# DonsetPG/graph-physics

Hardware: AMD Instinct MI355X
Metric: training steps/sec, CylinderFlow 15-round MGN (batch 16 meshes per step) (higher is better)
Workload: dtype f32; 1 GPU; BASELINE.json configs[1], fp32: 16 x 1885-node CylinderFlow-like meshes per GPU (N=30160, E=180082), 15 rounds, latent 128, random init; global_batch_meshes=16, launch=eager, parallelism=single

## Files before the change

graph-physics_amd/_capi.py:

```python
from __future__ import annotations

import ctypes as C
import os
import subprocess
import threading

_HERE = os.path.dirname(os.path.abspath(__file__))
_CSRC = os.path.join(_HERE, "csrc")
_REPO = os.path.dirname(_HERE)
LIB_PATH = os.environ.get("MGN_LIB") or os.path.join(_CSRC, "libmgn_hip.so")
SOURCES = [os.path.join(_CSRC, "mgn_kernels.hip"), os.path.join(_CSRC, "mgn_prep.hip"), os.path.join(_CSRC, "mgn_attn.hip"),
           os.path.join(_CSRC, "mgn_dense.hip"), os.path.join(_CSRC, "mgn_loss.hip")]
DEPS = [os.path.join(_CSRC, "mgn_x6.inc"), os.path.join(_CSRC, "mgn_fused.inc"), os.path.join(_CSRC, "mgn_pp.inc"), os.path.join(_CSRC, "mgn_ppr.inc")]
HEADER = os.path.join(_REPO, "include", "mgn_hip.h")
DEVICE_FLAGS = ["-Xclang", "-target-feature", "-Xclang", "-packed-fp32-ops"]

MAX_LAYERS = 8
MAX_PHASES = 3
MAX_WGRAD_JOBS = 48

_f32p = C.c_void_p
_i32p = C.c_void_p


class MlpFwdArgs(C.Structure):
    _fields_ = [
        ("M", C.c_int64),
        ("H", C.c_int), ("NL", C.c_int), ("nphase", C.c_int),
        ("src", _f32p * MAX_PHASES),
        ("idx", _i32p * MAX_PHASES),
        ("kw", C.c_int * MAX_PHASES),
        ("W", _f32p * MAX_LAYERS),
        ("b", _f32p * MAX_LAYERS),
        ("scale", _f32p),
        ("eps", C.c_float),
# ... 210 lines not shown
    "mgn_sparse_attn_fwd_s": (C.c_int, [C.c_void_p, C.c_int64] * 3 + [C.c_int, C.c_void_p, C.c_void_p, C.c_int64, C.c_int, C.c_int] + [C.c_void_p] * 4),
    "mgn_sparse_attn_bwd_s": (C.c_int, [C.c_void_p, C.c_int64] * 3 + [C.c_int] + [C.c_void_p] * 8 + [C.c_int64, C.c_int64, C.c_int, C.c_int]
                              + [C.c_void_p, C.c_int64] * 3 + [C.c_void_p, C.c_size_t, C.c_void_p]),
    "mgn_sparse_attn_weights": (C.c_int, [C.c_void_p] * 6 + [C.c_int64, C.c_int, C.c_int, C.c_void_p, C.c_void_p]),
    "mgn_head_axis_attn_fwd": (C.c_int, [C.c_void_p] * 3 + [C.c_int64, C.c_int, C.c_int] + [C.c_void_p] * 3),
    "mgn_head_axis_attn_bwd": (C.c_int, [C.c_void_p] * 6 + [C.c_int64, C.c_int, C.c_int] + [C.c_void_p] * 4),
    "mgn_attn_last_error": (C.c_char_p, []),
    "mgn_linear_fwd": (C.c_int, [C.POINTER(LinearArgs), C.c_void_p]),
    "mgn_linear_accepts_transposed": (C.c_int, [C.c_int64, C.c_int, C.c_int, C.c_int, C.c_int]),
    "mgn_rownorm2_bwd": (C.c_int, [C.c_void_p, C.c_void_p, C.c_int, C.c_int, C.c_void_p, C.c_void_p, C.c_void_p, C.c_void_p, C.c_float, C.c_int64,
                                   C.c_void_p, C.c_void_p, C.c_void_p, C.c_void_p, C.c_size_t, C.c_void_p]),
    "mgn_act_gate_bwd": (C.c_int, [C.c_void_p, C.c_void_p, C.c_void_p, C.c_int64, C.c_int, C.c_int, C.c_int, C.c_void_p, C.c_void_p, C.c_void_p]),
    "mgn_rownorm_fwd": (C.c_int, [C.c_void_p, C.c_int, C.c_int, C.c_void_p, C.c_float, C.c_int64, C.c_void_p, C.c_void_p, C.c_void_p]),
    "mgn_rownorm_bwd_workspace_bytes": (C.c_size_t, [C.c_int]),
    "mgn_rownorm_bwd": (C.c_int, [C.c_void_p, C.POINTER(RownormPhase), C.c_int, C.c_void_p, C.c_void_p, C.c_float, C.c_int64, C.c_void_p,
                                  C.c_void_p, C.c_size_t, C.c_void_p]),
    "mgn_dense_last_error": (C.c_char_p, []),
    "mgn_loss_fd_geometry": (C.c_int, [C.c_void_p] * 4 + [C.c_int, C.c_int64, C.c_void_p, C.c_void_p, C.c_void_p]),
    "mgn_loss_ls_geometry": (C.c_int, [C.c_void_p, C.c_int64, C.c_int, C.c_void_p, C.c_int, C.c_int64] + [C.c_void_p] * 6),
    "mgn_loss_workspace_bytes": (C.c_size_t, []),
    "mgn_loss_fwd": (C.c_int, [C.POINTER(LossArgs), C.c_void_p]),
    "mgn_loss_bwd": (C.c_int, [C.POINTER(LossArgs)] + [C.c_void_p] * 5),
    "mgn_loss_last_error": (C.c_char_p, []),
}

_lib = None
_lock = threading.Lock()

EXPECTED_VERSION = 136
HASH_PATH = os.path.join(_CSRC, "libmgn_hip.srchash")
LOCK_PATH = os.path.join(_CSRC, ".build.lock")


def hipcc_path():
    for p in (os.environ.get("HIPCC"), "/opt/rocm/bin/hipcc"):
        if p and os.path.exists(p):
            return p
    from shutil import which

    return which("hipcc")


def source_hash() -> str:
    import hashlib

    h = hashlib.sha256()
# ... 57 lines not shown
            if needs_build():
                try:
                    build()
                except Exception as e:
                    raise RuntimeError(
                        f"MI355X engine library {LIB_PATH} is missing or older than its sources and could not be "
                        f"rebuilt ({e}); run `python -c 'import __graft_entry__ as g; g.build()'`") from e
            try:
                L = C.CDLL(LIB_PATH)
            except OSError as e:
                raise RuntimeError(f"cannot load {LIB_PATH}: {e}") from e
            for name, (res, args) in SYMBOLS.items():
                fn = getattr(L, name)
                fn.restype = res
                fn.argtypes = args
            v = L.mgn_version()
            if v != EXPECTED_VERSION:
                raise RuntimeError(f"{LIB_PATH} has ABI version {v}, this binding needs {EXPECTED_VERSION}: rebuild it "
                                   "(`python -c 'import __graft_entry__ as g; g.build()'`)")
            _lib = L
    return _lib


def check(rc: int, what: str, prep: bool = False, attn: bool = False, dense: bool = False, loss: bool = False):
    if rc != 0:
        fn = lib().mgn_loss_last_error if loss else lib().mgn_dense_last_error if dense else (lib().mgn_attn_last_error if attn else (lib().mgn_prep_last_error if prep else lib().mgn_last_error))
        msg = fn().decode("utf-8", "replace")
        raise RuntimeError(f"{what} failed (code {rc}): {msg}")
```

graph-physics_amd/csrc/mgn_prep.hip:

```cpp
#include <hip/hip_runtime.h>
#include <rocprim/device/device_radix_sort.hpp>
#include <rocprim/device/device_select.hpp>
#include <stdint.h>
#include <stdio.h>
#include "mgn_hip.h"

static thread_local char g_perr[256] = "";
extern "C" const char* mgn_prep_last_error(void) { return g_perr; }
static int pfail(int code, const char* msg) {
  snprintf(g_perr, sizeof(g_perr), "%s", msg);
  return code;
}
static int pcheck(const char* what) {
  hipError_t e = hipGetLastError();
  if (e != hipSuccess) {
    snprintf(g_perr, sizeof(g_perr), "%s: %s", what, hipGetErrorString(e));
    return 2;
  }
  return 0;
}

__global__ void k_face_keys(const int64_t* __restrict__ face, int K, long F, long N, uint64_t* __restrict__ keys, int* __restrict__ err) {
  const long f = (long)blockIdx.x * blockDim.x + threadIdx.x;
  if (f >= F) return;
// ... 351 lines not shown

__device__ __forceinline__ float sim_value(const mgn_sim_desc& d, int stream, long row, int col) {
  if (stream == 0) {
    const int nf = d.feat_end - d.feat_start;
    if (col < nf) return d.x[row * d.x_w + d.feat_start + col];
    const float t = d.x[row * d.x_w + d.type_idx];
    const int ti = (int)(long)t;
    if (col == nf && d.type_err != nullptr && (ti < 0 || ti >= MGN_NODE_TYPES)) *d.type_err = 1;
    return (ti == col - nf) ? 1.f : 0.f;
  }
  if (stream == 1) return d.y[row * d.y_w + col] - d.x[row * d.x_w + d.out_start + col];
  return d.edge_attr[row * d.edge_w + col];
}
__device__ __forceinline__ int sim_width(const mgn_sim_desc& d, int stream) {
  return stream == 0 ? (d.feat_end - d.feat_start) + MGN_NODE_TYPES : stream == 1 ? d.out_w : d.edge_w;
}
__device__ __forceinline__ long sim_rows(const mgn_sim_desc& d, int stream) { return stream == 2 ? d.E : d.N; }

__global__ void __launch_bounds__(256) k_stats_partial(const mgn_sim_desc d, float* __restrict__ part) {
  const int stream = blockIdx.y;
  if (!d.accumulate[stream] || !(*d.num_acc[stream] < d.max_accumulations)) return;
  const int W = sim_width(d, stream);
  const long M = sim_rows(d, stream);
  __shared__ float s1[256], s2[256];
  const int col = threadIdx.x % SIM_MAXW, rl = threadIdx.x / SIM_MAXW;
  float a = 0.f, b = 0.f;
  if (col < W)
    for (long r = (long)blockIdx.x * 8 + rl; r < M; r += (long)SIM_PART * 8) {
      const float v = sim_value(d, stream, r, col);
      a += v;
      b = fmaf(v, v, b);
    }
  s1[threadIdx.x] = a;
  s2[threadIdx.x] = b;
  __syncthreads();
  if (rl == 0) {
    for (int k = 1; k < 8; ++k) {
      a += s1[k * SIM_MAXW + col];
      b += s2[k * SIM_MAXW + col];
    }
    float* p = part + ((size_t)(stream * SIM_PART + blockIdx.x) * 2) * SIM_MAXW;
    p[col] = a;
    p[SIM_MAXW + col] = b;
  }
}

__global__ void __launch_bounds__(64) k_stats_final(const mgn_sim_desc d, const float* __restrict__ part) {
  const int stream = blockIdx.x;
  if (!d.accumulate[stream] || !(*d.num_acc[stream] < d.max_accumulations)) return;
  const int W = sim_width(d, stream);
  const int col = threadIdx.x % SIM_MAXW, which = threadIdx.x / SIM_MAXW;
  if (col < W) {
    float t = 0.f;
    for (int b = 0; b < SIM_PART; ++b) t += part[((size_t)(stream * SIM_PART + b) * 2 + which) * SIM_MAXW + col];
    float* dst = which == 0 ? d.acc_sum[stream] : d.acc_sumsq[stream];
    dst[col] += t;
  }
  if (threadIdx.x == 0) {
    *d.acc_count[stream] += (float)sim_rows(d, stream);
// ... 663 lines not shown
```

graph-physics_amd/ops.py:

```python
from __future__ import annotations

import ctypes as C
from typing import List, Optional, Sequence, Tuple

import torch

from . import _capi

EPS = 1e-8
import os as _os
X6_ENABLED = _os.environ.get("MGN_FP32_MFMA") is None

_matrix_precision = "fp32"


def set_matrix_precision(p: str) -> None:
    global _matrix_precision
    if p not in ("fp32", "bf16"):
        raise ValueError("matrix precision must be 'fp32' or 'bf16'")
    if p == "bf16" and not X6_ENABLED:
        raise RuntimeError("bf16 matrix mode runs on the split-bf16 kernels; unset MGN_FP32_MFMA")
    _matrix_precision = p


def get_matrix_precision() -> str:
    return _matrix_precision
SUPPORTED_H = (16, 32, 64, 128)


def _ptr(t: Optional[torch.Tensor]) -> Optional[int]:
    return None if t is None else t.data_ptr()


_raw_stream = getattr(torch._C, "_cuda_getCurrentRawStream", None)
# ... 452 lines not shown

def wpack(blocks: Sequence[Tuple[int, int, bool, int]], dev):
    if not blocks:
        return
    arr = (_capi.WpackBlock * len(blocks))()
    for i, (src, ld, tr, dst) in enumerate(blocks):
        arr[i].src, arr[i].ld_src, arr[i].transpose, arr[i].dst = src, ld, int(bool(tr)), dst
    with torch.cuda.device(dev):
        rc = _capi.lib().mgn_wpack(len(blocks), arr, _stream(dev))
    _capi.check(rc, "mgn_wpack")


def transpose_blocks(blocks: Sequence[Tuple[int, int, int, int]], H: int, dev):
    if not blocks:
        return
    arr = (_capi.TBlock * len(blocks))()
    for i, (src, lds, dst, ldd) in enumerate(blocks):
        arr[i].src, arr[i].ld_src, arr[i].dst, arr[i].ld_dst = src, lds, dst, ldd
    with torch.cuda.device(dev):
        rc = _capi.lib().mgn_transpose_blocks(len(blocks), arr, H, _stream(dev))
    _capi.check(rc, "mgn_transpose_blocks")


def gather_rows(src: torch.Tensor, idx: torch.Tensor, out: Optional[torch.Tensor] = None) -> torch.Tensor:
    n, H = int(idx.numel()), int(src.shape[1])
    if out is None:
        out = torch.empty(n, H, dtype=torch.float32, device=src.device)
    with torch.cuda.device(src.device):
        rc = _capi.lib().mgn_gather_rows(_ptr(src), _ptr(idx), n, H, _ptr(out), _stream(src.device))
    _capi.check(rc, "mgn_gather_rows", prep=True)
    return out


def halo_unpack_add(rows: torch.Tensor, nodes: torch.Tensor, rowptr: torch.Tensor, perm: torch.Tensor, dst: torch.Tensor):
    with torch.cuda.device(dst.device):
        rc = _capi.lib().mgn_halo_unpack_add(_ptr(rows), _ptr(nodes), _ptr(rowptr), _ptr(perm), int(nodes.numel()), int(dst.shape[1]),
                                             _ptr(dst), _stream(dst.device))
    _capi.check(rc, "mgn_halo_unpack_add", prep=True)


def gate_fwd(G, phi, gate_pos, agg, gate_out, agg_out):
    with torch.cuda.device(agg.device):
        rc = _capi.lib().mgn_gate_fwd(_ptr(G), _ptr(phi), _ptr(gate_pos), _ptr(agg), int(agg.shape[0]), int(agg.shape[1]),
                                      _ptr(gate_out), _ptr(agg_out), _stream(agg.device))
    _capi.check(rc, "mgn_gate_fwd", prep=True)

# ... 150 lines not shown
    fit = int(frac * free // max(per_round, 1))
    return max(0, L - fit)


class MlpFunction(torch.autograd.Function):

    @staticmethod
    def forward(ctx, x, has_norm, act, *params):
        _require_device(x, *params)
        x = _f32c(x)
        NL = (len(params) - (1 if has_norm else 0)) // 2
        Ws = [_f32c(params[2 * l]) for l in range(NL)]
        bs = [_f32c(params[2 * l + 1]) for l in range(NL)]
        scale = _f32c(params[2 * NL]) if has_norm else None
        if NL < 2:
            raise AssertionError("The MLP must have at least 2 layers (input and output).")
        M, kin = x.shape
        H = Ws[0].shape[0]
        out_w = Ws[-1].shape[0]
        if H not in SUPPORTED_H or kin > H or out_w > H:
            raise NotImplementedError(f"MLP widths (in={kin}, hidden={H}, out={out_w}) not supported by the MI355X engine")
        dev = x.device
        kp, op = pad16(kin), pad16(out_w)
        W0 = Ws[0]
        if kp != kin:
            W0 = torch.nn.functional.pad(W0, (0, kp - kin))
        Wl, bl = Ws[-1], bs[-1]
        if op != out_w:
            Wl = torch.nn.functional.pad(Wl, (0, 0, 0, op - out_w))
            bl = torch.nn.functional.pad(bl, (0, op - out_w))
        Wk = [W0] + Ws[1:-1] + [Wl]
        bk = bs[:-1] + [bl]
        prec = 1 if (_matrix_precision == "bf16" and not (H == 128 and out_w == H and X6_ENABLED and act != 2)) else 0
        if prec:
            Wk = [w.to(torch.bfloat16).to(torch.float32) for w in Wk]
            bk = [b.to(torch.bfloat16).to(torch.float32) for b in bk]
        need = any(ctx.needs_input_grad) and _saving()
        f = dict(dtype=torch.float32, device=dev)
        y = torch.empty(M, out_w, **f)
        x6 = H == 128 and out_w == H and X6_ENABLED and M > 0 and act != 2
        mode = "generic"
        if x6 and kin < H and 3 <= NL <= 4:
            mode = "enc"
        elif x6 and kin == H and NL <= 4:
            mode = "full"
        packed = mode != "generic"
        saveH = [torch.empty(M, H, **f) for _ in range(NL - 1)] if need else None
        U = torch.empty(M, H, **f) if (need and has_norm) else None
        R = torch.empty(M, **f) if (need and has_norm) else None
        Ms = [torch.empty(M, 4, dtype=torch.int32, device=dev) for _ in range(NL - 1)] if (need and packed and act == 0) else None
        Zs = [torch.empty(M, H, **f) for _ in range(NL - 1)] if (need and act != 0) else None
        if mode == "enc":
            h1 = saveH[0] if need else torch.empty(M, H, **f)
            mlp_fwd(M, H, [(x, None, kin)], [Wk[0]], [bk[0]], None, H, None, h1, Zs[0] if Zs else None, out_relu=True, act=act,
                    saveM=[Ms[0]] if Ms else None)
            pk = torch.empty((NL - 1) * _capi.WPACK_BYTES, dtype=torch.uint8, device=dev)
            units = [pk.data_ptr() + u * _capi.WPACK_BYTES for u in range(NL - 1)]
            wpack([(Wk[l + 1].data_ptr(), H, False, units[l]) for l in range(NL - 1)], dev)
            mlp_fwd(M, H, [(h1, None, H)], Wk[1:], bk[1:], scale, out_w, None, y, None,
                    saveH[1:] if need else None, U, R, wpk=units, saveM=Ms[1:] if Ms else None,
                    saveZ=Zs[1:] if Zs else None, act=act)
        elif mode == "full":
            pk = torch.empty(NL * _capi.WPACK_BYTES, dtype=torch.uint8, device=dev)
            units = [pk.data_ptr() + u * _capi.WPACK_BYTES for u in range(NL)]
            wpack([(Wk[l].data_ptr(), H, False, units[l]) for l in range(NL)], dev)
            mlp_fwd(M, H, [(x, None, H)], Wk, bk, scale, out_w, None, y, None, saveH, U, R, wpk=units, saveM=Ms, saveZ=Zs, act=act)
        else:
            mlp_fwd(M, H, [(x, None, kin)], Wk, bk, scale, out_w, None, y, None, saveH, U, R, act=act, saveZ=Zs, precision=prec)
        ctx.meta = (NL, H, kin, out_w, has_norm, kp != kin, op != out_w, act, mode)
        ctx.prec, ctx.Wk_rounded = prec, (Wk if prec else None)
        ctx.save_for_backward(x, *Ws, *([scale] if has_norm else []))
        ctx.pads = (W0 if kp != kin else None, Wl if op != out_w else None)
        ctx.saved_acts = (saveH, U, R, Ms, Zs)
        return y

    @staticmethod
    def backward(ctx, dy):
        NL, H, kin, out_w, has_norm, pad0, padl, act, mode = ctx.meta
        if ctx.saved_acts is None or ctx.saved_acts[0] is None:
            raise RuntimeError("MlpFunction: no saved activations -- backward ran a second time without retain_graph "
                               "support, or the forward ran under no_grad")
        t = ctx.saved_tensors
        x, Ws = t[0], list(t[1:1 + NL])
        scale = t[1 + NL] if has_norm else None
        Wk = [ctx.pads[0] if pad0 else Ws[0]] + Ws[1:-1] + [ctx.pads[1] if padl else Ws[-1]]
        prec = getattr(ctx, "prec", 0)
        if prec:
            Wk = ctx.Wk_rounded
        saveH, U, R, Ms, Zs = ctx.saved_acts
        dy = _f32c(dy)
        M, dev = x.shape[0], x.device
        kp, op = pad16(kin), pad16(out_w)
        f = dict(dtype=torch.float32, device=dev)
        widths = [H] * (NL - 1) + [op]
        zero = M == 0
        mk = torch.zeros if zero else torch.empty
        dZ = [mk(M, w, **f) for w in widths]
        db = [mk(w, **f) for w in widths]
        dscale = mk(H, **f) if has_norm else None
        dx = None
        want_dx = ctx.needs_input_grad[0]
        if want_dx and kin != H:
            raise NotImplementedError("input gradient of a ragged-width MLP input is not needed by the path")
        if want_dx:
            dx = mk(M, H, **f)
        if mode in ("enc", "full") and M > 0:
            tr = [Wk[l] for l in range(NL - 1, 0, -1)] + ([Wk[0]] if want_dx else [])
            pk = torch.empty(len(tr) * _capi.WPACK_BYTES, dtype=torch.uint8, device=dev)
            units = [pk.data_ptr() + u * _capi.WPACK_BYTES for u in range(len(tr))]
            wpack([(w.data_ptr(), H, True, units[u]) for u, w in enumerate(tr)], dev)
            din = [(None, None, dx)] if want_dx else []
            mlp_bwd(M, H, NL, dy, None, None, out_w, U, R, scale, saveH, [None] * NL, dZ, din, [None] * NL, dscale,
                    wpk=units, Ms=Ms, Zs=Zs, act=act)
        else:
            sq = [l for l in range(1, NL) if tuple(Wk[l].shape) == (H, H) and Wk[l].is_contiguous()]
            wt_buf = torch.empty(len(sq), H, H, **f) if sq else None
            if sq:
                transpose_blocks([(Wk[l].data_ptr(), H, wt_buf[k].data_ptr(), H) for k, l in enumerate(sq)], H, dev)
            WT = [None] + [wt_buf[sq.index(l)] if l in sq else Wk[l].t().contiguous() for l in range(1, NL)]
            din = [(Wk[0].t().contiguous(), None, dx)] if want_dx else []
            mlp_bwd(M, H, NL, dy, None, None, out_w, U, R, scale, saveH, WT, dZ, din, [None] * NL, dscale, act=act, Zs=Zs, precision=prec)
        ins = [x.to(torch.bfloat16).to(torch.float32) if prec else x] + list(saveH)
        in_w = [kin] + [H] * (NL - 1)
        dWs = [mk(widths[l], in_w[l], **f) for l in range(NL)]
        jobs = []
        for l in range(NL):
            jobs.append((dZ[l], widths[l], widths[l] // 16, ins[l], in_w[l], pad16(in_w[l]) // 16, in_w[l], dWs[l], 0, in_w[l], db[l]))
        if M > 0:
            wgrad(jobs, dev)
        grads = []
        for l in range(NL):
            dW, dbl = dWs[l], db[l]
            if l == NL - 1 and op != out_w:
                dW, dbl = dW[:out_w], dbl[:out_w]
            grads += [dW, dbl]
        if has_norm:
            grads.append(dscale)
        ctx.saved_acts = None
        return (dx, None, None, *grads)


def _split_block(q, spec: BlockSpec):
    NL, k = spec.nb_layers, spec.mlp_params
    We, be = [q[2 * l] for l in range(NL)], [q[2 * l + 1] for l in range(NL)]
    se = q[2 * NL] if spec.layer_norm else None
    Wn, bn = [q[k + 2 * l] for l in range(NL)], [q[k + 2 * l + 1] for l in range(NL)]
    sn = q[k + 2 * NL] if spec.layer_norm else None
    gp_ = tuple(q[2 * k: 2 * k + 3]) if spec.gate else None
    return We, be, se, Wn, bn, sn, gp_


class ProcessorFunction(torch.autograd.Function):

    @staticmethod
    def forward(ctx, x, e, topo: Topology, L: int, spec: BlockSpec, halo, pos, phi, rope_inv_freq, *params):
        _require_device(x, e, *params)
# ... 498 lines not shown
```

include/mgn_hip.h:

```cpp
#ifndef MGN_HIP_H
#define MGN_HIP_H

#include <stddef.h>
#include <stdint.h>

#ifdef __cplusplus
extern "C" {
#endif

#define MGN_MAX_LAYERS 8
#define MGN_MAX_PHASES 3
#define MGN_MAX_WGRAD_JOBS 48

int mgn_version(void);
const char* mgn_last_error(void);

size_t mgn_csr_workspace_bytes(int64_t E, int64_t N);
int mgn_csr_build(const int64_t* key, int64_t E, int64_t N, int32_t* rowptr, int32_t* perm,
                  void* ws, size_t ws_bytes, void* stream);

size_t mgn_topology_workspace_bytes(int64_t E, int64_t N);
int mgn_topology_build(const int64_t* src, const int64_t* dst, int64_t E, int64_t N, int32_t* rowptr_dst, int32_t* perm_dst,
                       int32_t* src_s, int32_t* dst_s, int32_t* rowptr_src, int32_t* perm_src, int32_t* max_degree_host,
                       void* ws, size_t ws_bytes, void* stream);
// ... 326 lines not shown
  const float* type; int ldty;
  float types[4]; int ntypes;
  int nterms; int term_type[MGN_LOSS_MAX_TERMS]; float term_weight[MGN_LOSS_MAX_TERMS];
  const int64_t* rowptr; const int32_t* col; const float* coef;
  const float* inv;
  int64_t M; int K;
  const int32_t* elems; const float* cv;
  const int64_t* nptr; const int32_t* nent;
  float* ge_out; float* ge_tgt;
  float* g_out;
  float* a_out; float* bu_out; float* b_out;
  float* part;
  float* terms; float* total; float* invcount;
} mgn_loss_args;
int mgn_loss_fd_geometry(const int64_t* rowptr, const int32_t* col, const uint8_t* self_loop, const float* pos, int DX, int64_t N,
                         float* coef, float* inv, void* stream);
int mgn_loss_ls_geometry(const int32_t* elems, int64_t M, int K, const float* pos, int DX, int64_t N, const int64_t* nptr,
                         const int32_t* nent, float* cv, double* vol, float* inv, void* stream);
size_t mgn_loss_workspace_bytes(void);
int mgn_loss_fwd(const mgn_loss_args* args, void* stream);
int mgn_loss_bwd(const mgn_loss_args* args, const float* g, float* d_net, float* d_u, float* dge, void* stream);
const char* mgn_loss_last_error(void);

#ifdef __cplusplus
}
#endif
#endif
```

Measured before the change: 81.70 steps/s.

## Add narrow-width kernels for encoder input and decoder output MLP layers

Adds dedicated HIP kernels for the encoder's first layer (small input width up to 16) and the decoder's last layer (small output width). Each has fused forward, ReLU-mask, dH and weight-gradient passes, with partial-sum reductions. This replaces padded 16-wide tiles in the generic MLP and wgrad path, and a new 'dec' mode runs three packed hidden layers plus a narrow output layer. It aims to cut wasted padded compute and memory traffic on the thin layers, at the cost of more code paths and extra reduction launches.

Result: faster. 82.54 steps/s, median of 6 (+1.0%).

```diff
diff --git a/graph-physics_amd/_capi.py b/graph-physics_amd/_capi.py
--- a/graph-physics_amd/_capi.py
+++ b/graph-physics_amd/_capi.py
@@ -10,7 +10,7 @@
 _REPO = os.path.dirname(_HERE)
 LIB_PATH = os.environ.get("MGN_LIB") or os.path.join(_CSRC, "libmgn_hip.so")
 SOURCES = [os.path.join(_CSRC, "mgn_kernels.hip"), os.path.join(_CSRC, "mgn_prep.hip"), os.path.join(_CSRC, "mgn_attn.hip"),
-           os.path.join(_CSRC, "mgn_dense.hip"), os.path.join(_CSRC, "mgn_loss.hip")]
+           os.path.join(_CSRC, "mgn_dense.hip"), os.path.join(_CSRC, "mgn_loss.hip"), os.path.join(_CSRC, "mgn_narrow.hip")]
 DEPS = [os.path.join(_CSRC, "mgn_x6.inc"), os.path.join(_CSRC, "mgn_fused.inc"), os.path.join(_CSRC, "mgn_pp.inc"), os.path.join(_CSRC, "mgn_ppr.inc")]
 HEADER = os.path.join(_REPO, "include", "mgn_hip.h")
 DEVICE_FLAGS = ["-Xclang", "-target-feature", "-Xclang", "-packed-fp32-ops"]
@@ -267,6 +267,14 @@
     "mgn_loss_fwd": (C.c_int, [C.POINTER(LossArgs), C.c_void_p]),
     "mgn_loss_bwd": (C.c_int, [C.POINTER(LossArgs)] + [C.c_void_p] * 5),
     "mgn_loss_last_error": (C.c_char_p, []),
+    "mgn_narrow_fwd_in": (C.c_int, [C.c_void_p, C.c_int, C.c_int, C.c_void_p, C.c_int, C.c_void_p, C.c_int64, C.c_void_p, C.c_void_p, C.c_int, C.c_void_p]),
+    "mgn_narrow_wgrad_in_workspace_bytes": (C.c_size_t, [C.c_int64, C.c_int]),
+    "mgn_narrow_wgrad_in": (C.c_int, [C.c_void_p, C.c_void_p, C.c_int, C.c_int, C.c_int64, C.c_void_p, C.c_int, C.c_void_p, C.c_void_p, C.c_size_t, C.c_void_p]),
+    "mgn_narrow_fwd_out": (C.c_int, [C.c_void_p, C.c_void_p, C.c_void_p, C.c_int, C.c_int64, C.c_void_p, C.c_int, C.c_int, C.c_void_p]),
+    "mgn_narrow_bwd_out_workspace_bytes": (C.c_size_t, [C.c_int64, C.c_int]),
+    "mgn_narrow_bwd_out": (C.c_int, [C.c_void_p, C.c_int, C.c_int, C.c_void_p, C.c_void_p, C.c_void_p, C.c_int, C.c_int64, C.c_void_p, C.c_void_p, C.c_void_p, C.c_void_p,
+                                     C.c_size_t, C.c_void_p]),
+    "mgn_narrow_last_error": (C.c_char_p, []),
 }
 
 _lib = None
@@ -370,8 +378,8 @@
     return _lib
 
 
-def check(rc: int, what: str, prep: bool = False, attn: bool = False, dense: bool = False, loss: bool = False):
+def check(rc: int, what: str, prep: bool = False, attn: bool = False, dense: bool = False, loss: bool = False, narrow: bool = False):
     if rc != 0:
-        fn = lib().mgn_loss_last_error if loss else lib().mgn_dense_last_error if dense else (lib().mgn_attn_last_error if attn else (lib().mgn_prep_last_error if prep else lib().mgn_last_error))
+        fn = lib().mgn_narrow_last_error if narrow else lib().mgn_loss_last_error if loss else lib().mgn_dense_last_error if dense else (lib().mgn_attn_last_error if attn else (lib().mgn_prep_last_error if prep else lib().mgn_last_error))
         msg = fn().decode("utf-8", "replace")
         raise RuntimeError(f"{what} failed (code {rc}): {msg}")
diff --git a/graph-physics_amd/csrc/mgn_narrow.hip b/graph-physics_amd/csrc/mgn_narrow.hip
--- /dev/null
+++ b/graph-physics_amd/csrc/mgn_narrow.hip
@@ -0,0 +1,334 @@
+#include <hip/hip_runtime.h>
+#include <stdint.h>
+#include <stdio.h>
+#include "mgn_hip.h"
+
+static thread_local char g_nerr[256] = "";
+extern "C" const char* mgn_narrow_last_error(void) { return g_nerr; }
+static int nfail(int code, const char* msg) {
+  snprintf(g_nerr, sizeof(g_nerr), "%s", msg);
+  return code;
+}
+static int ncheck(const char* what) {
+  hipError_t e = hipGetLastError();
+  if (e != hipSuccess) {
+    snprintf(g_nerr, sizeof(g_nerr), "%s: %s", what, hipGetErrorString(e));
+    return 2;
+  }
+  return 0;
+}
+
+#define NARROW_H 128
+#define NARROW_MAXW 16
+#define NARROW_WG_MAX 1024
+#define NARROW_OS 132
+
+template <int KP>
+__global__ void __launch_bounds__(256) k_narrow_fwd_in(const float* __restrict__ x, int ldx, int kin, const float* __restrict__ W,
+                                                       int ldw, const float* __restrict__ b, long M, float* __restrict__ h,
+                                                       uint32_t* __restrict__ mask, int relu) {
+  const int lane = threadIdx.x & 63, q = lane & 31, half = lane >> 5;
+  float w[4][KP], bias[4];
+#pragma unroll
+  for (int r = 0; r < 4; ++r) {
+    bias[r] = b != nullptr ? b[4 * q + r] : 0.f;
+#pragma unroll
+    for (int k = 0; k < KP; ++k) w[r][k] = (k < kin) ? W[(long)(4 * q + r) * ldw + k] : 0.f;
+  }
+  const long wave = (long)blockIdx.x * 4 + (threadIdx.x >> 6), nwave = (long)gridDim.x * 4;
+  for (long r0 = wave * 8; r0 < M; r0 += nwave * 8) {
+#pragma unroll
+    for (int i = 0; i < 4; ++i) {
+      const long m = r0 + 2 * i + half;
+      const bool ok = m < M;
+      const float* xr = x + (ok ? m : M - 1) * ldx;
+      float xv[KP];
+#pragma unroll
+      for (int k = 0; k < KP; ++k) xv[k] = (k < kin) ? xr[k] : 0.f;
+      float z[4];
+      uint32_t bits = 0;
+#pragma unroll
+      for (int r = 0; r < 4; ++r) {
+        float t = bias[r];
+#pragma unroll
+        for (int ks = 0; ks < 4; ++ks)
+#pragma unroll
+          for (int kg = 0; kg < KP / 4; ++kg) t = fmaf(w[r][4 * kg + ks], xv[4 * kg + ks], t);
+        if (relu) {
+          t = fmaxf(t, 0.f);
+          bits |= (t > 0.f) ? (1u << (4 * (q >> 2) + r)) : 0u;
+        }
+        z[r] = t;
+      }
+      if (ok) *(float4*)(h + m * NARROW_H + 4 * q) = make_float4(z[0], z[1], z[2], z[3]);
+      if (mask != nullptr) {
+        bits |= __shfl_xor(bits, 4);
+        bits |= __shfl_xor(bits, 8);
+        bits |= __shfl_xor(bits, 16);
+        if (ok && q < 4) mask[m * 4 + q] = bits;
+      }
+    }
+  }
+}
+
+template <int KP>
+__global__ void __launch_bounds__(256) k_narrow_wgrad_in(const float* __restrict__ dZ, const float* __restrict__ x, int ldx, int kin,
+                                                         long M, float* __restrict__ part) {
+  constexpr int NE = NARROW_H * (KP + 1);
+  __shared__ float red[NE];
+  const int q = threadIdx.x & 31, hw = threadIdx.x >> 5;
+  float acc[4][KP], s[4];
+#pragma unroll
+  for (int r = 0; r < 4; ++r) {
+    s[r] = 0.f;
+#pragma unroll
+    for (int k = 0; k < KP; ++k) acc[r][k] = 0.f;
+  }
+  const long ghw = (long)blockIdx.x * 8 + hw, nhw = (long)gridDim.x * 8;
+  for (long m0 = ghw * 4; m0 < M; m0 += nhw * 4) {
+#pragma unroll
+    for (int i = 0; i < 4; ++i) {
+      const long m = m0 + i;
+      const bool ok = m < M;
+      const long mc = ok ? m : M - 1;
+      const float4 d4 = *(const float4*)(dZ + mc * NARROW_H + 4 * q);
+      const float d[4] = {ok ? d4.x : 0.f, ok ? d4.y : 0.f, ok ? d4.z : 0.f, ok ? d4.w : 0.f};
+      float xv[KP];
+#pragma unroll
+      for (int k = 0; k < KP; ++k) xv[k] = (ok && k < kin) ? x[mc * ldx + k] : 0.f;
+#pragma unroll
+      for (int r = 0; r < 4; ++r) {
+        s[r] += d[r];
+#pragma unroll
+        for (int k = 0; k < KP; ++k) acc[r][k] = fmaf(d[r], xv[k], acc[r][k]);
+      }
+    }
+  }
+  for (int sel = 0; sel < 8; ++sel) {
+    if (hw == sel) {
+#pragma unroll
+      for (int r = 0; r < 4; ++r) {
+        float* p = red + (4 * q + r) * (KP + 1);
+#pragma unroll
+        for (int k = 0; k < KP; ++k) p[k] = (sel == 0 ? 0.f : p[k]) + acc[r][k];
+        p[KP] = (sel == 0 ? 0.f : p[KP]) + s[r];
+      }
+    }
+    __syncthreads();
+  }
+  float* dst = part + (size_t)blockIdx.x * NE;
+  for (int t = threadIdx.x; t < NE; t += 256) dst[t] = red[t];
+}
+
+__global__ void __launch_bounds__(256) k_narrow_wgrad_red(const float* __restrict__ part, int nwg, int pstride, int nelem, int ne1, int kout,
+                                                          float* __restrict__ dW, int ldw, float* __restrict__ db) {
+  __shared__ float sh[256];
+  const int el = threadIdx.x & 15, sl = threadIdx.x >> 4;
+  const int e = blockIdx.x * 16 + el;
+  float a = 0.f;
+  if (e < nelem)
+    for (int w = sl; w < nwg; w += 16) a += part[(size_t)w * pstride + e];
+  sh[threadIdx.x] = a;
+  __syncthreads();
+  if (sl == 0 && e < nelem) {
+    for (int k = 1; k < 16; ++k) a += sh[k * 16 + el];
+    const int j = e / ne1, k = e % ne1;
+    if (k == ne1 - 1) {
+      if (db != nullptr) db[j] = a;
+    } else if (k < kout) {
+      dW[(long)j * ldw + k] = a;
+    }
+  }
+}
+
+template <int OP>
+__global__ void __launch_bounds__(256) k_narrow_fwd_out(const float* __restrict__ h, const float* __restrict__ W, const float* __restrict__ b,
+                                                        int out, long M, float* __restrict__ y, int ldy, int relu_in) {
+  const int lane = threadIdx.x & 63, q = lane & 31, half = lane >> 5;
+  float4 w[OP];
+#pragma unroll
+  for (int o = 0; o < OP; ++o) w[o] = (o < out) ? *(const float4*)(W + o * NARROW_H + 4 * q) : make_float4(0.f, 0.f, 0.f, 0.f);
+  const float bq = (b != nullptr && q < out) ? b[q] : 0.f;
+  const long wave = (long)blockIdx.x * 4 + (threadIdx.x >> 6), nwave = (long)gridDim.x * 4;
+  for (long r0 = wave * 8; r0 < M; r0 += nwave * 8) {
+#pragma unroll
+    for (int i = 0; i < 4; ++i) {
+      const long m = r0 + 2 * i + half;
+      const bool ok = m < M;
+      float4 v = *(const float4*)(h + (ok ? m : M - 1) * NARROW_H + 4 * q);
+      if (relu_in) v = make_float4(fmaxf(v.x, 0.f), fmaxf(v.y, 0.f), fmaxf(v.z, 0.f), fmaxf(v.w, 0.f));
+      float mine = 0.f;
+#pragma unroll
+      for (int o = 0; o < OP; ++o) {
+        float t = fmaf(w[o].x, v.x, fmaf(w[o].y, v.y, fmaf(w[o].z, v.z, w[o].w * v.w)));
+        t += __shfl_xor(t, 16);
+        t += __shfl_xor(t, 8);
+        t += __shfl_xor(t, 4);
+        t += __shfl_xor(t, 2);
+        t += __shfl_xor(t, 1);
+        if (q == o) mine = t;
+      }
+      if (ok && q < out) y[m * ldy + q] = mine + bq;
+    }
+  }
+}
+
+template <int OP>
+__global__ void __launch_bounds__(256) k_narrow_bwd_out(const float* __restrict__ dy, int ldy, int out, const float* __restrict__ W,
+                                                        const float* __restrict__ h, const uint32_t* __restrict__ mask, int relu_in, long M,
+                                                        float* __restrict__ dH, float* __restrict__ part) {
+  constexpr int NE = OP * NARROW_OS;
+  __shared__ __attribute__((aligned(16))) float red[NE];
+  const int q = threadIdx.x & 31, hw = threadIdx.x >> 5;
+  float4 w[OP], acc[OP];
+  float s[OP];
+#pragma unroll
+  for (int o = 0; o < OP; ++o) {
+    w[o] = (o < out) ? *(const float4*)(W + o * NARROW_H + 4 * q) : make_float4(0.f, 0.f, 0.f, 0.f);
+    acc[o] = make_float4(0.f, 0.f, 0.f, 0.f);
+    s[o] = 0.f;
+  }
+  const long ghw = (long)blockIdx.x * 8 + hw, nhw = (long)gridDim.x * 8;
+  for (long m0 = ghw * 4; m0 < M; m0 += nhw * 4) {
+#pragma unroll
+    for (int i = 0; i < 4; ++i) {
+      const long m = m0 + i;
+      const bool ok = m < M;
+      const long mc = ok ? m : M - 1;
+      const float4 hv4 = *(const float4*)(h + mc * NARROW_H + 4 * q);
+      float4 hv = ok ? hv4 : make_float4(0.f, 0.f, 0.f, 0.f);
+      uint32_t bits = mask != nullptr ? (mask[mc * 4 + (q & 3)] >> (4 * (q >> 2))) & 15u : 15u;
+      if (relu_in) {
+        bits = (hv.x > 0.f ? 1u : 0u) | (hv.y > 0.f ? 2u : 0u) | (hv.z > 0.f ? 4u : 0u) | (hv.w > 0.f ? 8u : 0u);
+        hv = make_float4(fmaxf(hv.x, 0.f), fmaxf(hv.y, 0.f), fmaxf(hv.z, 0.f), fmaxf(hv.w, 0.f));
+      }
+      float4 g = make_float4(0.f, 0.f, 0.f, 0.f);
+#pragma unroll
+      for (int o = 0; o < OP; ++o) {
+        const float d = (ok && o < out) ? dy[mc * ldy + o] : 0.f;
+        g.x = fmaf(d, w[o].x, g.x), g.y = fmaf(d, w[o].y, g.y), g.z = fmaf(d, w[o].z, g.z), g.w = fmaf(d, w[o].w, g.w);
+        acc[o].x = fmaf(d, hv.x, acc[o].x), acc[o].y = fmaf(d, hv.y, acc[o].y);
+        acc[o].z = fmaf(d, hv.z, acc[o].z), acc[o].w = fmaf(d, hv.w, acc[o].w);
+        s[o] += d;
+      }
+      if (ok)
+        *(float4*)(dH + m * NARROW_H + 4 * q) =
+            make_float4((bits & 1u) ? g.x : 0.f, (bits & 2u) ? g.y : 0.f, (bits & 4u) ? g.z : 0.f, (bits & 8u) ? g.w : 0.f);
+    }
+  }
+  for (int sel = 0; sel < 8; ++sel) {
+    if (hw == sel) {
+#pragma unroll
+      for (int o = 0; o < OP; ++o) {
+        float* p = red + o * NARROW_OS;
+        const float4 old = sel == 0 ? make_float4(0.f, 0.f, 0.f, 0.f) : *(const float4*)(p + 4 * q);
+        *(float4*)(p + 4 * q) = make_float4(old.x + acc[o].x, old.y + acc[o].y, old.z + acc[o].z, old.w + acc[o].w);
+        if (q == 0) p[NARROW_OS - 1] = (sel == 0 ? 0.f : p[NARROW_OS - 1]) + s[o];
+      }
+    }
+    __syncthreads();
+  }
+  float* dst = part + (size_t)blockIdx.x * NE;
+  for (int t = threadIdx.x; t < NE; t += 256) dst[t] = red[t];
+}
+
+static unsigned wgrad_grid(int64_t M) {
+  const int64_t g = (M + 31) / 32;
+  return (unsigned)(g < 1 ? 1 : (g > NARROW_WG_MAX ? NARROW_WG_MAX : g));
+}
+static unsigned fwd_grid(int64_t M) {
+  const int64_t g = (M + 31) / 32;
+  return (unsigned)(g < 1 ? 1 : (g > 4096 ? 4096 : g));
+}
+static bool aligned16(const void* p) { return ((uintptr_t)p & 15u) == 0; }
+
+extern "C" int mgn_narrow_fwd_in(const float* x, int ldx, int kin, const float* W, int ldw, const float* b, int64_t M, float* h,
+                                 void* mask, int relu, void* stream) {
+  if (kin < 1 || kin > NARROW_MAXW || ldx < kin || ldw < kin || M < 0) return nfail(1, "mgn_narrow_fwd_in: 1 <= kin <= 16, ldx >= kin, ldw >= kin");
+  if (M == 0) return 0;
+  if (x == nullptr || W == nullptr || h == nullptr || !aligned16(h)) return nfail(1, "mgn_narrow_fwd_in: null or misaligned operand");
+  if (mask != nullptr && !relu) return nfail(1, "mgn_narrow_fwd_in: sign-bit words are those of a ReLU");
+  hipStream_t s = (hipStream_t)stream;
+  const dim3 grid(fwd_grid(M)), block(256);
+  uint32_t* mk = (uint32_t*)mask;
+  switch ((kin + 3) / 4) {
+    case 1: hipLaunchKernelGGL(k_narrow_fwd_in<4>, grid, block, 0, s, x, ldx, kin, W, ldw, b, (long)M, h, mk, relu); break;
+    case 2: hipLaunchKernelGGL(k_narrow_fwd_in<8>, grid, block, 0, s, x, ldx, kin, W, ldw, b, (long)M, h, mk, relu); break;
+    case 3: hipLaunchKernelGGL(k_narrow_fwd_in<12>, grid, block, 0, s, x, ldx, kin, W, ldw, b, (long)M, h, mk, relu); break;
+    default: hipLaunchKernelGGL(k_narrow_fwd_in<16>, grid, block, 0, s, x, ldx, kin, W, ldw, b, (long)M, h, mk, relu); break;
+  }
+  return ncheck("mgn_narrow_fwd_in");
+}
+
+extern "C" size_t mgn_narrow_wgrad_in_workspace_bytes(int64_t M, int kin) {
+  if (M <= 0 || kin < 1 || kin > NARROW_MAXW) return 0;
+  const int KP = 4 * ((kin + 3) / 4);
+  return (size_t)wgrad_grid(M) * NARROW_H * (KP + 1) * sizeof(float);
+}
+
+extern "C" int mgn_narrow_wgrad_in(const float* dZ, const float* x, int ldx, int kin, int64_t M, float* dW, int ldw, float* db, void* ws,
+                                   size_t ws_bytes, void* stream) {
+  if (kin < 1 || kin > NARROW_MAXW || ldx < kin || ldw < kin || M < 1) return nfail(1, "mgn_narrow_wgrad_in: 1 <= kin <= 16, ldx >= kin, ldw >= kin, M >= 1");
+  if (dZ == nullptr || x == nullptr || dW == nullptr || !aligned16(dZ)) return nfail(1, "mgn_narrow_wgrad_in: null or misaligned operand");
+  if (ws == nullptr || ws_bytes < mgn_narrow_wgrad_in_workspace_bytes(M, kin)) return nfail(1, "mgn_narrow_wgrad_in: workspace too small");
+  hipStream_t s = (hipStream_t)stream;
+  const unsigned nwg = wgrad_grid(M);
+  const dim3 grid(nwg), block(256);
+  float* part = (float*)ws;
+  const int KP = 4 * ((kin + 3) / 4);
+  switch (KP) {
+    case 4: hipLaunchKernelGGL(k_narrow_wgrad_in<4>, grid, block, 0, s, dZ, x, ldx, kin, (long)M, part); break;
+    case 8: hipLaunchKernelGGL(k_narrow_wgrad_in<8>, grid, block, 0, s, dZ, x, ldx, kin, (long)M, part); break;
+    case 12: hipLaunchKernelGGL(k_narrow_wgrad_in<12>, grid, block, 0, s, dZ, x, ldx, kin, (long)M, part); break;
+    default: hipLaunchKernelGGL(k_narrow_wgrad_in<16>, grid, block, 0, s, dZ, x, ldx, kin, (long)M, part); break;
+  }
+  const int nelem = NARROW_H * (KP + 1);
+  hipLaunchKernelGGL(k_narrow_wgrad_red, dim3((nelem + 15) / 16), block, 0, s, (const float*)part, (int)nwg, nelem, nelem, KP + 1, kin, dW, ldw, db);
+  return ncheck("mgn_narrow_wgrad_in");
+}
+
+extern "C" int mgn_narrow_fwd_out(const float* h, const float* W, const float* b, int out, int64_t M, float* y, int ldy, int relu_in,
+                                  void* stream) {
+  if (out < 1 || out > NARROW_MAXW || ldy < out || M < 0) return nfail(1, "mgn_narrow_fwd_out: 1 <= out <= 16, ldy >= out");
+  if (M == 0) return 0;
+  if (h == nullptr || W == nullptr || y == nullptr || !aligned16(h) || !aligned16(W)) return nfail(1, "mgn_narrow_fwd_out: null or misaligned operand");
+  hipStream_t s = (hipStream_t)stream;
+  const dim3 grid(fwd_grid(M)), block(256);
+  switch ((out + 3) / 4) {
+    case 1: hipLaunchKernelGGL(k_narrow_fwd_out<4>, grid, block, 0, s, h, W, b, out, (long)M, y, ldy, relu_in); break;
+    case 2: hipLaunchKernelGGL(k_narrow_fwd_out<8>, grid, block, 0, s, h, W, b, out, (long)M, y, ldy, relu_in); break;
+    case 3: hipLaunchKernelGGL(k_narrow_fwd_out<12>, grid, block, 0, s, h, W, b, out, (long)M, y, ldy, relu_in); break;
+    default: hipLaunchKernelGGL(k_narrow_fwd_out<16>, grid, block, 0, s, h, W, b, out, (long)M, y, ldy, relu_in); break;
+  }
+  return ncheck("mgn_narrow_fwd_out");
+}
+
+extern "C" size_t mgn_narrow_bwd_out_workspace_bytes(int64_t M, int out) {
+  if (M <= 0 || out < 1 || out > NARROW_MAXW) return 0;
+  const int OP = 4 * ((out + 3) / 4);
+  return (size_t)wgrad_grid(M) * OP * NARROW_OS * sizeof(float);
+}
+
+extern "C" int mgn_narrow_bwd_out(const float* dy, int ldy, int out, const float* W, const float* h, const void* mask, int relu_in, int64_t M,
+                                  float* dH, float* dW, float* db, void* ws, size_t ws_bytes, void* stream) {
+  if (out < 1 || out > NARROW_MAXW || ldy < out || M < 1) return nfail(1, "mgn_narrow_bwd_out: 1 <= out <= 16, ldy >= out, M >= 1");
+  if (dy == nullptr || W == nullptr || h == nullptr || dH == nullptr || dW == nullptr || !aligned16(h) || !aligned16(W) || !aligned16(dH))
+    return nfail(1, "mgn_narrow_bwd_out: null or misaligned operand");
+  if (ws == nullptr || ws_bytes < mgn_narrow_bwd_out_workspace_bytes(M, out)) return nfail(1, "mgn_narrow_bwd_out: workspace too small");
+  hipStream_t s = (hipStream_t)stream;
+  const unsigned nwg = wgrad_grid(M);
+  const dim3 grid(nwg), block(256);
+  float* part = (float*)ws;
+  const uint32_t* mk = (const uint32_t*)mask;
+  const int OP = 4 * ((out + 3) / 4);
+  switch (OP) {
+    case 4: hipLaunchKernelGGL(k_narrow_bwd_out<4>, grid, block, 0, s, dy, ldy, out, W, h, mk, relu_in, (long)M, dH, part); break;
+    case 8: hipLaunchKernelGGL(k_narrow_bwd_out<8>, grid, block, 0, s, dy, ldy, out, W, h, mk, relu_in, (long)M, dH, part); break;
+    case 12: hipLaunchKernelGGL(k_narrow_bwd_out<12>, grid, block, 0, s, dy, ldy, out, W, h, mk, relu_in, (long)M, dH, part); break;
+    default: hipLaunchKernelGGL(k_narrow_bwd_out<16>, grid, block, 0, s, dy, ldy, out, W, h, mk, relu_in, (long)M, dH, part); break;
+  }
+  const int nelem = out * NARROW_OS;
+  hipLaunchKernelGGL(k_narrow_wgrad_red, dim3((nelem + 15) / 16), block, 0, s, (const float*)part, (int)nwg, OP * NARROW_OS, nelem,
+                     NARROW_OS, NARROW_H, dW, NARROW_H, db);
+  return ncheck("mgn_narrow_bwd_out");
+}
diff --git a/graph-physics_amd/csrc/mgn_prep.hip b/graph-physics_amd/csrc/mgn_prep.hip
--- a/graph-physics_amd/csrc/mgn_prep.hip
+++ b/graph-physics_amd/csrc/mgn_prep.hip
@@ -397,19 +397,34 @@
   if (!d.accumulate[stream] || !(*d.num_acc[stream] < d.max_accumulations)) return;
   const int W = sim_width(d, stream);
   const long M = sim_rows(d, stream);
-  __shared__ float s1[256], s2[256];
-  const int col = threadIdx.x % SIM_MAXW, rl = threadIdx.x / SIM_MAXW;
-  float a = 0.f, b = 0.f;
-  if (col < W)
-    for (long r = (long)blockIdx.x * 8 + rl; r < M; r += (long)SIM_PART * 8) {
+  __shared__ float s1[8 * SIM_MAXW], s2[8 * SIM_MAXW];
+  if (W < 1) return;
+  const int col = threadIdx.x % W, rl = threadIdx.x / W;
+  if (rl < 8) {
+    float a = 0.f, b = 0.f;
+    const long step = (long)SIM_PART * 8;
+    long r = (long)blockIdx.x * 8 + rl;
+    for (; r + 7 * step < M; r += 8 * step) {
+      float v[8];
+#pragma unroll
+      for (int i = 0; i < 8; ++i) v[i] = sim_value(d, stream, r + i * step, col);
+#pragma unroll
+      for (int i = 0; i < 8; ++i) {
+        a += v[i];
+        b = fmaf(v[i], v[i], b);
+      }
+    }
+    for (; r < M; r += step) {
       const float v = sim_value(d, stream, r, col);
       a += v;
       b = fmaf(v, v, b);
     }
-  s1[threadIdx.x] = a;
-  s2[threadIdx.x] = b;
+    s1[rl * SIM_MAXW + col] = a;
+    s2[rl * SIM_MAXW + col] = b;
+  }
   __syncthreads();
   if (rl == 0) {
+    float a = s1[col], b = s2[col];
     for (int k = 1; k < 8; ++k) {
       a += s1[k * SIM_MAXW + col];
       b += s2[k * SIM_MAXW + col];
diff --git a/graph-physics_amd/ops.py b/graph-physics_amd/ops.py
--- a/graph-physics_amd/ops.py
+++ b/graph-physics_amd/ops.py
@@ -10,6 +10,8 @@
 EPS = 1e-8
 import os as _os
 X6_ENABLED = _os.environ.get("MGN_FP32_MFMA") is None
+STEP_TAIL = _os.environ.get("MGN_STEP_TAIL", "1") != "0"
+NARROW_FWD = _os.environ.get("MGN_NARROW_FWD", "0") == "1"
 
 _matrix_precision = "fp32"
 
@@ -508,6 +510,46 @@
     _capi.check(rc, "mgn_transpose_blocks")
 
 
+def narrow_fwd_in(x: torch.Tensor, W: torch.Tensor, b: Optional[torch.Tensor], h: torch.Tensor, mask: Optional[torch.Tensor] = None,
+                  relu: bool = True):
+    M, kin = x.shape
+    dev = x.device
+    with torch.cuda.device(dev):
+        rc = _capi.lib().mgn_narrow_fwd_in(_ptr(x), x.stride(0), kin, _ptr(W), W.stride(0), _ptr(b), M, _ptr(h), _ptr(mask), int(relu), _stream(dev))
+    _capi.check(rc, "mgn_narrow_fwd_in", narrow=True)
+
+
+def narrow_wgrad_in(dZ: torch.Tensor, x: torch.Tensor, dW: torch.Tensor, db: Optional[torch.Tensor]):
+    M, kin = x.shape
+    if M == 0:
+        return
+    L, dev = _capi.lib(), x.device
+    ws = torch.empty(max(L.mgn_narrow_wgrad_in_workspace_bytes(M, kin), 16), dtype=torch.uint8, device=dev)
+    with torch.cuda.device(dev):
+        rc = L.mgn_narrow_wgrad_in(_ptr(dZ), _ptr(x), x.stride(0), kin, M, _ptr(dW), dW.stride(0), _ptr(db), _ptr(ws), ws.numel(), _stream(dev))
+    _capi.check(rc, "mgn_narrow_wgrad_in", narrow=True)
+
+
+def narrow_fwd_out(h: torch.Tensor, W: torch.Tensor, b: Optional[torch.Tensor], y: torch.Tensor, relu_in: bool = False):
+    M, dev = h.shape[0], h.device
+    with torch.cuda.device(dev):
+        rc = _capi.lib().mgn_narrow_fwd_out(_ptr(h), _ptr(W), _ptr(b), W.shape[0], M, _ptr(y), y.stride(0), int(relu_in), _stream(dev))
+    _capi.check(rc, "mgn_narrow_fwd_out", narrow=True)
+
+
+def narrow_bwd_out(dy: torch.Tensor, W: torch.Tensor, h: torch.Tensor, mask: Optional[torch.Tensor], dH: torch.Tensor, dW: torch.Tensor,
+                   db: Optional[torch.Tensor], relu_in: bool = False):
+    M, dev = h.shape[0], h.device
+    if M == 0:
+        return
+    L, out = _capi.lib(), W.shape[0]
+    ws = torch.empty(max(L.mgn_narrow_bwd_out_workspace_bytes(M, out), 16), dtype=torch.uint8, device=dev)
+    with torch.cuda.device(dev):
+        rc = L.mgn_narrow_bwd_out(_ptr(dy), dy.stride(0), out, _ptr(W), _ptr(h), _ptr(mask), int(relu_in), M, _ptr(dH), _ptr(dW), _ptr(db),
+                                  _ptr(ws), ws.numel(), _stream(dev))
+    _capi.check(rc, "mgn_narrow_bwd_out", narrow=True)
+
+
 def gather_rows(src: torch.Tensor, idx: torch.Tensor, out: Optional[torch.Tensor] = None) -> torch.Tensor:
     n, H = int(idx.numel()), int(src.shape[1])
     if out is None:
@@ -704,11 +746,22 @@
             raise NotImplementedError(f"MLP widths (in={kin}, hidden={H}, out={out_w}) not supported by the MI355X engine")
         dev = x.device
         kp, op = pad16(kin), pad16(out_w)
+        x6 = H == 128 and X6_ENABLED and M > 0 and act != 2
+        mode = "generic"
+        if x6 and out_w == H and kin < H and 3 <= NL <= 4:
+            mode = "enc"
+        elif x6 and out_w == H and kin == H and NL <= 4:
+            mode = "full"
+        elif (x6 and STEP_TAIL and kin == H and out_w <= 16 and NL == 4 and not has_norm and act == 0
+              and _matrix_precision != "bf16"):
+            mode = "dec"
+        narrow_in = STEP_TAIL and mode == "enc" and act == 0 and kin <= 16
+        narrow_fwd = narrow_in and NARROW_FWD
         W0 = Ws[0]
-        if kp != kin:
+        if kp != kin and not narrow_fwd:
             W0 = torch.nn.functional.pad(W0, (0, kp - kin))
         Wl, bl = Ws[-1], bs[-1]
-        if op != out_w:
+        if op != out_w and mode != "dec":
             Wl = torch.nn.functional.pad(Wl, (0, 0, 0, op - out_w))
             bl = torch.nn.functional.pad(bl, (0, op - out_w))
         Wk = [W0] + Ws[1:-1] + [Wl]
@@ -720,22 +773,20 @@
         need = any(ctx.needs_input_grad) and _saving()
         f = dict(dtype=torch.float32, device=dev)
         y = torch.empty(M, out_w, **f)
-        x6 = H == 128 and out_w == H and X6_ENABLED and M > 0 and act != 2
-        mode = "generic"
-        if x6 and kin < H and 3 <= NL <= 4:
-            mode = "enc"
-        elif x6 and kin == H and NL <= 4:
-            mode = "full"
         packed = mode != "generic"
-        saveH = [torch.empty(M, H, **f) for _ in range(NL - 1)] if need else None
+        nsave = NL - 2 if mode == "dec" else NL - 1
+        saveH = [torch.empty(M, H, **f) for _ in range(nsave)] if need else None
         U = torch.empty(M, H, **f) if (need and has_norm) else None
         R = torch.empty(M, **f) if (need and has_norm) else None
-        Ms = [torch.empty(M, 4, dtype=torch.int32, device=dev) for _ in range(NL - 1)] if (need and packed and act == 0) else None
+        Ms = [torch.empty(M, 4, dtype=torch.int32, device=dev) for _ in range(nsave)] if (need and packed and act == 0) else None
         Zs = [torch.empty(M, H, **f) for _ in range(NL - 1)] if (need and act != 0) else None
         if mode == "enc":
             h1 = saveH[0] if need else torch.empty(M, H, **f)
-            mlp_fwd(M, H, [(x, None, kin)], [Wk[0]], [bk[0]], None, H, None, h1, Zs[0] if Zs else None, out_relu=True, act=act,
-                    saveM=[Ms[0]] if Ms else None)
+            if narrow_fwd:
+                narrow_fwd_in(x, Wk[0], bk[0], h1, Ms[0] if Ms else None)
+            else:
+                mlp_fwd(M, H, [(x, None, kin)], [Wk[0]], [bk[0]], None, H, None, h1, Zs[0] if Zs else None, out_relu=True, act=act,
+                        saveM=[Ms[0]] if Ms else None)
             pk = torch.empty((NL - 1) * _capi.WPACK_BYTES, dtype=torch.uint8, device=dev)
             units = [pk.data_ptr() + u * _capi.WPACK_BYTES for u in range(NL - 1)]
             wpack([(Wk[l + 1].data_ptr(), H, False, units[l]) for l in range(NL - 1)], dev)
@@ -747,12 +798,21 @@
             units = [pk.data_ptr() + u * _capi.WPACK_BYTES for u in range(NL)]
             wpack([(Wk[l].data_ptr(), H, False, units[l]) for l in range(NL)], dev)
             mlp_fwd(M, H, [(x, None, H)], Wk, bk, scale, out_w, None, y, None, saveH, U, R, wpk=units, saveM=Ms, saveZ=Zs, act=act)
+        elif mode == "dec":
+            pk = torch.empty(3 * _capi.WPACK_BYTES, dtype=torch.uint8, device=dev)
+            units = [pk.data_ptr() + u * _capi.WPACK_BYTES for u in range(3)]
+            wpack([(Wk[l].data_ptr(), H, False, units[l]) for l in range(3)], dev)
+            z3 = torch.empty(M, H, **f)
+            mlp_fwd(M, H, [(x, None, H)], Wk[:3], bk[:3], None, H, None, z3, None, saveH, None, None, wpk=units, saveM=Ms)
+            narrow_fwd_out(z3, Wk[3], bk[3], y, relu_in=True)
+            Zs = [z3] if need else None
         else:
             mlp_fwd(M, H, [(x, None, kin)], Wk, bk, scale, out_w, None, y, None, saveH, U, R, act=act, saveZ=Zs, precision=prec)
-        ctx.meta = (NL, H, kin, out_w, has_norm, kp != kin, op != out_w, act, mode)
+        ctx.meta = (NL, H, kin, out_w, has_norm, kp != kin and not narrow_fwd, op != out_w and mode != "dec", act, mode)
+        ctx.narrow_in = narrow_in
         ctx.prec, ctx.Wk_rounded = prec, (Wk if prec else None)
         ctx.save_for_backward(x, *Ws, *([scale] if has_norm else []))
-        ctx.pads = (W0 if kp != kin else None, Wl if op != out_w else None)
+        ctx.pads = (W0 if kp != kin and not narrow_fwd else None, Wl if op != out_w and mode != "dec" else None)
         ctx.saved_acts = (saveH, U, R, Ms, Zs)
         return y
 
@@ -774,10 +834,11 @@
         M, dev = x.shape[0], x.device
         kp, op = pad16(kin), pad16(out_w)
         f = dict(dtype=torch.float32, device=dev)
-        widths = [H] * (NL - 1) + [op]
+        dec = mode == "dec"
+        widths = [H] * (NL - 1) + [out_w if dec else op]
         zero = M == 0
         mk = torch.zeros if zero else torch.empty
-        dZ = [mk(M, w, **f) for w in widths]
+        dZ = [mk(M, w, **f) if not (dec and l == NL - 1) else None for l, w in enumerate(widths)]
         db = [mk(w, **f) for w in widths]
         dscale = mk(H, **f) if has_norm else None
         dx = None
@@ -786,7 +847,18 @@
             raise NotImplementedError("input gradient of a ragged-width MLP input is not needed by the path")
         if want_dx:
             dx = mk(M, H, **f)
-        if mode in ("enc", "full") and M > 0:
+        in_w = [kin] + [H] * (NL - 1)
+        dWs = [mk(widths[l], in_w[l], **f) for l in range(NL)]
+        if dec and M > 0:
+            narrow_bwd_out(dy, Wk[3], Zs[0], None, dZ[2], dWs[3], db[3], relu_in=True)
+            tr = [Wk[2], Wk[1]] + ([Wk[0]] if want_dx else [])
+            pk = torch.empty(len(tr) * _capi.WPACK_BYTES, dtype=torch.uint8, device=dev)
+            units = [pk.data_ptr() + u * _capi.WPACK_BYTES for u in range(len(tr))]
+            wpack([(w.data_ptr(), H, True, units[u]) for u, w in enumerate(tr)], dev)
+            din = [(None, None, dx)] if want_dx else []
+            mlp_bwd(M, H, 3, dZ[2], None, None, H, None, None, None, saveH, [None] * 3, [dZ[0], dZ[1], None], din, [None] * 3, None,
+                    wpk=units, Ms=Ms)
+        elif mode in ("enc", "full") and M > 0:
             tr = [Wk[l] for l in range(NL - 1, 0, -1)] + ([Wk[0]] if want_dx else [])
             pk = torch.empty(len(tr) * _capi.WPACK_BYTES, dtype=torch.uint8, device=dev)
             units = [pk.data_ptr() + u * _capi.WPACK_BYTES for u in range(len(tr))]
@@ -794,7 +866,7 @@
             din = [(None, None, dx)] if want_dx else []
             mlp_bwd(M, H, NL, dy, None, None, out_w, U, R, scale, saveH, [None] * NL, dZ, din, [None] * NL, dscale,
                     wpk=units, Ms=Ms, Zs=Zs, act=act)
-        else:
+        elif not dec:
             sq = [l for l in range(1, NL) if tuple(Wk[l].shape) == (H, H) and Wk[l].is_contiguous()]
             wt_buf = torch.empty(len(sq), H, H, **f) if sq else None
             if sq:
@@ -803,17 +875,19 @@
             din = [(Wk[0].t().contiguous(), None, dx)] if want_dx else []
             mlp_bwd(M, H, NL, dy, None, None, out_w, U, R, scale, saveH, WT, dZ, din, [None] * NL, dscale, act=act, Zs=Zs, precision=prec)
         ins = [x.to(torch.bfloat16).to(torch.float32) if prec else x] + list(saveH)
-        in_w = [kin] + [H] * (NL - 1)
-        dWs = [mk(widths[l], in_w[l], **f) for l in range(NL)]
         jobs = []
         for l in range(NL):
+            if (dec and l == NL - 1) or (ctx.narrow_in and l == 0):
+                continue
             jobs.append((dZ[l], widths[l], widths[l] // 16, ins[l], in_w[l], pad16(in_w[l]) // 16, in_w[l], dWs[l], 0, in_w[l], db[l]))
         if M > 0:
+            if ctx.narrow_in:
+                narrow_wgrad_in(dZ[0], x, dWs[0], db[0])
             wgrad(jobs, dev)
         grads = []
         for l in range(NL):
             dW, dbl = dWs[l], db[l]
-            if l == NL - 1 and op != out_w:
+            if l == NL - 1 and op != out_w and not dec:
                 dW, dbl = dW[:out_w], dbl[:out_w]
             grads += [dW, dbl]
         if has_norm:
diff --git a/include/mgn_hip.h b/include/mgn_hip.h
--- a/include/mgn_hip.h
+++ b/include/mgn_hip.h
@@ -372,6 +372,17 @@
 int mgn_loss_bwd(const mgn_loss_args* args, const float* g, float* d_net, float* d_u, float* dge, void* stream);
 const char* mgn_loss_last_error(void);
 
+int mgn_narrow_fwd_in(const float* x, int ldx, int kin, const float* W, int ldw, const float* b, int64_t M, float* h,
+                      void* mask, int relu, void* stream);
+size_t mgn_narrow_wgrad_in_workspace_bytes(int64_t M, int kin);
+int mgn_narrow_wgrad_in(const float* dZ, const float* x, int ldx, int kin, int64_t M, float* dW, int ldw, float* db, void* ws,
+                        size_t ws_bytes, void* stream);
+int mgn_narrow_fwd_out(const float* h, const float* W, const float* b, int out, int64_t M, float* y, int ldy, int relu_in, void* stream);
+size_t mgn_narrow_bwd_out_workspace_bytes(int64_t M, int out);
+int mgn_narrow_bwd_out(const float* dy, int ldy, int out, const float* W, const float* h, const void* mask, int relu_in, int64_t M,
+                       float* dH, float* dW, float* db, void* ws, size_t ws_bytes, void* stream);
+const char* mgn_narrow_last_error(void);
+
 #ifdef __cplusplus
 }
 #endif
```
